# trustbloc/fabric-mod

Measured on AMD Instinct MI355X. Metric: ECDSA P-256 verifies/sec (whole node), higher is better.
Workload: dtype int64; 1 GPU; BASELINE.json configs[1]: block of 10000 tx x 3 endorsements = 30000 P-256 tuples per GPU, verify-only kernel via the C ABI, fresh keypair per signatu; tuples_per_gpu=30000, tx_per_block=10000, endorsements_per_tx=3, seed=20260921, parallelism=1 block per GPU, clock_warmup_launches=100

## Files before the change

### fabric-mod_amd/csrc/fabgpu_api.hip

```cpp
#include <hip/hip_runtime.h>
#include <stdlib.h>
#include <string.h>

#include <algorithm>
#include <atomic>
#include <chrono>
#include <memory>
#include <sys/mman.h>
#include <set>
#include <mutex>
#include <new>
#include <map>
#include <string>
#include <thread>
#include <vector>

#include "../../include/fabgpu.h"
#include "kernels.h"
#include "block_walk_dev.h"
#include "worker_pool.h"
#include "bn_tables29.h"
#include "p256_tables29.h"

using namespace fab;
// ... 77 lines not shown
        cap = want;
        return FABGPU_OK;
    }
    void release() {
        if (h && is_huge) pinned_huge_free(h);
        else if (h) hipHostFree(h);
        h = nullptr;
        cap = 0;
        is_huge = false;
    }
};

}

struct fabgpu_ctx {
    int device = 0;
    bool allow_pair = true;
    bool allow_quad = true;
    bool nym_side_stream = true;
    std::atomic<bool> test_nym_side_after{false};
    bool nym_two_phase = true;
    bool allow_wide = true;
    int pair_table_lds = -1;
    hipStream_t stream = nullptr;
    int fault = 0;
    int32_t* d_gtab = nullptr;
    std::mutex mu;
    Buf fields;
    Buf arena;
    Buf offs;
    Buf out;
    hipEvent_t ev0 = nullptr, ev1 = nullptr;
    bool timed = false;
    bool time_kernels = false;
    struct QWs {
        void* p = nullptr;
        size_t bytes = 0;
        hipEvent_t done = nullptr;
        bool reserved = false;
        bool armed = false;
        NymSide nym_side;
        hipStream_t last = nullptr;
    };
    std::vector<QWs> qws;
    std::mutex kmu;
    std::vector<int32_t*> ktabs;
// ... 155 lines not shown
const char* fabgpu_strerror(int code) {
    switch (code) {
        case FABGPU_OK: return "ok";
        case FABGPU_EINVAL: return "invalid argument";
        case FABGPU_ENODEV: return "no usable gfx950 device (HIP runtime/device unavailable); fall back to bccsp/sw";
        case FABGPU_ENOMEM: return "host or device allocation failed";
        case FABGPU_ELAUNCH: return "HIP launch/copy/execution failure";
        case FABGPU_ETOOBIG: return "batch or arena exceeds 32-bit offsets";
        default: return "unknown fabgpu error";
    }
}

int fabgpu_device_count(fabgpu_ctx*) {
    int n = 0;
    if (hipGetDeviceCount(&n) != hipSuccess) return FABGPU_ENODEV;
    return n;
}

int fabgpu_init(const fabgpu_cfg* cfg, fabgpu_ctx** out) {
    if (!out) return FABGPU_EINVAL;
    *out = nullptr;
    if (cfg && (cfg->flags & ~(uint32_t)(FABGPU_FLAG_ONE_LANE_ONLY | FABGPU_FLAG_TIME_KERNELS | FABGPU_FLAG_NO_QUAD | FABGPU_FLAG_PAIR_TABLE_LDS |
                                          FABGPU_FLAG_PAIR_TABLE_GLOBAL | FABGPU_FLAG_NO_WIDE | FABGPU_FLAG_NYM_FUSED_HASH | FABGPU_FLAG_NYM_NO_SIDE_STREAM |
                                          FABGPU_FLAG_KEY_TABLES_16BIT)) != 0) return FABGPU_EINVAL;
    if (cfg && (cfg->flags & FABGPU_FLAG_PAIR_TABLE_LDS) && (cfg->flags & FABGPU_FLAG_PAIR_TABLE_GLOBAL)) return FABGPU_EINVAL;
    int ndev = 0;
    if (hipGetDeviceCount(&ndev) != hipSuccess || ndev <= 0) return FABGPU_ENODEV;
    int dev = cfg ? cfg->device : -1;
    if (dev < 0) {
        if (hipGetDevice(&dev) != hipSuccess) return FABGPU_ENODEV;
    }
    if (dev >= ndev) return FABGPU_EINVAL;
    hipDeviceProp_t prop;
    if (hipGetDeviceProperties(&prop, dev) != hipSuccess) return FABGPU_ENODEV;
    if (strncmp(prop.gcnArchName, "gfx950", 6) != 0) return FABGPU_ENODEV;
    fabgpu_ctx* ctx = new (std::nothrow) fabgpu_ctx();
    if (!ctx) return FABGPU_ENOMEM;
    ctx->device = dev;
    ctx->walk_map.flags = hipHostMallocMapped | hipHostMallocCoherent;
    ctx->allow_pair = !(cfg && (cfg->flags & FABGPU_FLAG_ONE_LANE_ONLY));
    ctx->allow_quad = !(cfg && (cfg->flags & FABGPU_FLAG_NO_QUAD));
    ctx->nym_two_phase = !(cfg && (cfg->flags & FABGPU_FLAG_NYM_FUSED_HASH));
    ctx->nym_side_stream = !(cfg && (cfg->flags & FABGPU_FLAG_NYM_NO_SIDE_STREAM));
    ctx->key_tables_16 = cfg && (cfg->flags & FABGPU_FLAG_KEY_TABLES_16BIT);
    ctx->allow_wide = ctx->allow_pair && !(cfg && (cfg->flags & FABGPU_FLAG_NO_WIDE));
    ctx->pair_table_lds = cfg && (cfg->flags & FABGPU_FLAG_PAIR_TABLE_LDS) ? 1 : (cfg && (cfg->flags & FABGPU_FLAG_PAIR_TABLE_GLOBAL) ? 0 : pair_table_default());
    if (std::max<size_t>(prop.sharedMemPerBlock, prop.maxSharedMemoryPerMultiProcessor) < pair_table_lds_bytes()) ctx->pair_table_lds = 0;
    ctx->time_kernels = cfg && (cfg->flags & FABGPU_FLAG_TIME_KERNELS);
    DeviceGuard g(dev);
    int rc = FABGPU_OK;
    do {
        if (hipStreamCreateWithFlags(&ctx->stream, hipStreamNonBlocking) != hipSuccess) { rc = FABGPU_ENODEV; break; }
        if (hipStreamCreateWithFlags(&ctx->stream2, hipStreamNonBlocking) != hipSuccess) { rc = FABGPU_ENODEV; break; }
        if (hipEventCreateWithFlags(&ctx->ev_up, hipEventDisableTiming) != hipSuccess) { rc = FABGPU_ENODEV; break; }
        if (hipStreamCreateWithFlags(&ctx->stream3, hipStreamNonBlocking) != hipSuccess) { rc = FABGPU_ENODEV; break; }
        if (hipStreamCreateWithFlags(&ctx->stream4, hipStreamNonBlocking) != hipSuccess) { rc = FABGPU_ENODEV; break; }
        if (hipStreamCreateWithFlags(&ctx->stream_copy, hipStreamNonBlocking) != hipSuccess) { rc = FABGPU_ENODEV; break; }
        {
            bool ok = true;
            for (auto& sc : ctx->stream_copy_more) ok = ok && hipStreamCreateWithFlags(&sc, hipStreamNonBlocking) == hipSuccess;
            if (!ok) { rc = FABGPU_ENODEV; break; }
        }
        {
            bool ok = true;
            for (auto& e : ctx->ev_w) ok = ok && hipEventCreateWithFlags(&e, hipEventDisableTiming) == hipSuccess;
            if (!ok) { rc = FABGPU_ENODEV; break; }
        }
        if (const char* fi = getenv("FABGPU_FAULT_INJECT")) ctx->fault = !strcmp(fi, "launch") ? 1 : (!strcmp(fi, "oom") ? 2 : 0);
        if (hipEventCreate(&ctx->ev0) != hipSuccess || hipEventCreate(&ctx->ev1) != hipSuccess) { rc = FABGPU_ENODEV; break; }
        if (hipMalloc((void**)&ctx->d_gtab, sizeof(int32_t) * GTab16::TABLE_WORDS) != hipSuccess) { rc = FABGPU_ENOMEM; break; }
// ... 111 lines not shown
}
float fab::ctx_last_kernel_ms(fabgpu_ctx* ctx) {
    if (!ctx || !ctx->timed) return -1.0f;
    DeviceGuard g(ctx->device);
    if (hipEventSynchronize(ctx->ev1) != hipSuccess) return -1.0f;
    float ms = -1.0f;
    if (hipEventElapsedTime(&ms, ctx->ev0, ctx->ev1) != hipSuccess) return -1.0f;
    return ms;
}
extern "C" {

int fabgpu_p256_verify_batch_dev(fabgpu_ctx* ctx, size_t n, const void* qx, const void* qy, const void* e, const void* r,
                                 const void* s, void* verdict_bits, void* status, void* stream) {
    if (!ctx || (n && (!qx || !qy || !e || !r || !s || !verdict_bits))) return FABGPU_EINVAL;
    if (n > 0xFFFFFFF0ull) return FABGPU_ETOOBIG;
    if (n == 0) return FABGPU_OK;
    DeviceGuard g(ctx->device);
    hipStream_t st = (hipStream_t)stream;
    size_t wi = 0;
    void* wsp = nullptr;
    int rc = ctx->acquire_qws(verify_workspace_bytes((uint32_t)n, ctx->allow_pair), &wi, &wsp, st);
    if (rc != FABGPU_OK) return rc;
    if (ctx->time_kernels) hipEventRecord(ctx->ev0, st);
    hipError_t err = launch_p256_verify((uint32_t)n, qx, qy, e, r, s, ctx->d_gtab, wsp, verdict_bits, status, ctx->allow_pair, st, 0, ctx->pair_table_lds);
    if (ctx->time_kernels) hipEventRecord(ctx->ev1, st);
    ctx->release_qws(wi, st);
    ctx->timed = ctx->time_kernels;
    return hip_to_rc(launched(ctx, err));
}

int fabgpu_sha256_batch_dev(fabgpu_ctx* ctx, size_t n, const void* arena, size_t arena_bytes, const void* off, void* digests,
                            void* stream) {
    if (!ctx || (n && (!arena || !off || !digests))) return FABGPU_EINVAL;
    if (n > 0xFFFFFFF0ull || arena_bytes > 0xFFFFFFFFull) return FABGPU_ETOOBIG;
    if (n == 0) return FABGPU_OK;
    DeviceGuard g(ctx->device);
    hipStream_t st = (hipStream_t)stream;
    if (ctx->time_kernels) hipEventRecord(ctx->ev0, st);
    hipError_t err = launch_sha256_batch((uint32_t)n, arena, arena_bytes, off, digests, st);
    if (ctx->time_kernels) hipEventRecord(ctx->ev1, st);
    ctx->timed = ctx->time_kernels;
    return hip_to_rc(launched(ctx, err));
}

int fabgpu_sha256_p256_verify_batch_dev(fabgpu_ctx* ctx, size_t n, const void* arena, size_t arena_bytes, const void* off,
                                        const void* qx, const void* qy, const void* r, const void* s, void* verdict_bits,
                                        void* status, void* stream) {
// ... 1842 lines not shown
        if (keyed) {
            e = launch_sha256_p256_verify_keyed(n, sl->d, arena_bytes, a.off2 + 2 * (size_t)row0, a.key_id + row0, nkeys, (const void*)kt, a.r + 32 * (size_t)row0,
                                                a.s + 32 * (size_t)row0, ctx->d_gtab, bits, dt + o_dst + row0, pair, p, ls);
        } else {
            size_t wi = 0;
            void* wsp = nullptr;
            int r2 = ctx->acquire_qws(verify_workspace_bytes(n, pair), &wi, &wsp, ls);
            if (r2 != FABGPU_OK) return r2;
            e = launch_sha256_p256_verify(n, sl->d, arena_bytes, a.off2 + 2 * (size_t)row0, a.qx + 32 * (size_t)row0, a.qy + 32 * (size_t)row0,
                                          a.r + 32 * (size_t)row0, a.s + 32 * (size_t)row0, ctx->d_gtab, wsp, bits, dt + o_dst + row0, pair, p, ls);
            ctx->release_qws(wi, ls);
        }
        return hip_to_rc(e);
    };
    auto verify_creators = [&](bool keyed) -> int {
        hipError_t e;
        if (keyed) {
            e = launch_p256_verify_keyed(tot.creators, a.key_id, nkeys, (const void*)kt, dt + o_dig, a.r, a.s, ctx->d_gtab, dt + o_bitc, dt + o_dst, true, s2, exclusive ? 84u << 10 : 0u);
        } else {
            size_t wi = 0;
            void* wsp = nullptr;
            int r2 = ctx->acquire_qws(verify_workspace_bytes(tot.creators, true), &wi, &wsp, s2);
            if (r2 != FABGPU_OK) return r2;
            e = launch_p256_verify(tot.creators, a.qx, a.qy, dt + o_dig, a.r, a.s, ctx->d_gtab, wsp, dt + o_bitc, dt + o_dst, true, s2, exclusive ? 84u << 10 : 0u, ctx->pair_table_lds);
            ctx->release_qws(wi, s2);
        }
        return hip_to_rc(e);
    };
    auto finish = [&]() -> int {
        if (++ctx->walk_seq == 0) ++ctx->walk_seq;
        ho.seq = ctx->walk_seq;
        if (err == hipSuccess && nym_ran) err = hipStreamWaitEvent(st, ctx->ev_w[6], 0);
        if (err == hipSuccess && memo) err = hipMemsetAsync(dt + o_mslots, 0, (size_t)out.memo_slot_cap * 4, st);
        if (err == hipSuccess && memo) err = hipMemsetAsync(&((WalkMemoTotals*)(dt + o_mtot))->live, 0, 4, st);
        mark("finish: memsets queued");
        if (!memo && !out.tuples && !out.tuple_digest && !out.tuple_qxy && !(has_nym_rows && out.nym_issuer) && walk_small_finish_fits(a, nc)) {
            if (err == hipSuccess) err = launch_walk_status_finish_small(a, nc, ho, st);
            mark("finish: last kernel queued");
            if (err != hipSuccess) return hip_to_rc(err);
            int r2 = wait_host_flag((const uint32_t*)(mh + m_finflag), ho.seq, st);
            if (r2 != FABGPU_OK) return r2;
            rq.summary = *(const WalkSummary*)(mh + m_sum);
            return FABGPU_OK;
        }
        if (err == hipSuccess) err = launch_walk_status_checks(a, nc, st);
        if (memo) {
            if (err == hipSuccess) err = launch_walk_memo_late(a, st);
// ... 335 lines not shown
```

### fabric-mod_amd/csrc/gputest.hip

```cpp
#include <hip/hip_runtime.h>
#include <stdint.h>

#include <vector>

#include "p256_pair29.h"
#include "pair29_bn_gcn.h"
#include "p256_tables29.h"
#include "bn_nym29.h"
#include "bn_quad29.h"
#include "bn_tables29.h"
#include "device_common.h"

using namespace fab;

__global__ void __launch_bounds__(64, 1) gputest_pair_kernel(int op, const int32_t* __restrict__ in, int32_t* __restrict__ out) {
    const int32_t* p = in + threadIdx.x * 36;
    pair_pt P;
    fe C, D;
    for (int i = 0; i < 9; i++) {
        P.A.v[i] = p[i];
        P.B.v[i] = p[9 + i];
        C.v[i] = p[18 + i];
        D.v[i] = p[27 + i];
    }
// ... 277 lines not shown
    hipEventCreate(&e0);
    hipEventCreate(&e1);
    hipLaunchKernelGGL(gputest_mac_ceiling_kernel, dim3(cus), dim3(threads), 0, 0, iters / 16 + 1, 12345u, d);
    hipDeviceSynchronize();
    hipEventRecord(e0, 0);
    hipLaunchKernelGGL(gputest_mac_ceiling_kernel, dim3(cus), dim3(threads), 0, 0, iters, 12345u, d);
    hipEventRecord(e1, 0);
    int rc = hipEventSynchronize(e1) == hipSuccess ? 0 : 4;
    float ms = 0;
    hipEventElapsedTime(&ms, e0, e1);
    std::vector<uint64_t> h(waves);
    if (rc == 0 && hipMemcpy(h.data(), d, sizeof(uint64_t) * waves, hipMemcpyDeviceToHost) != hipSuccess) rc = 5;
    double sum = 0;
    for (uint64_t v : h) sum += (double)v;
    out4[0] = ms;
    out4[1] = sum / waves;
    out4[2] = (double)waves * 64.0 * 64.0 * (double)iters;
    out4[3] = waves;
    hipEventDestroy(e0);
    hipEventDestroy(e1);
    hipFree(d);
    return rc;
}
```

### fabric-mod_amd/csrc/kernels.h

```cpp
#pragma once
#include <hip/hip_runtime_api.h>
#include <stddef.h>
#include <stdint.h>

namespace fab {
constexpr int KTAB_STRIDE = 2;
constexpr int VERIFY_BLOCK = 256;
constexpr int VERIFY_MAX_WGS = 256;
constexpr int VERIFY_PAIR_MAX = 32768;
constexpr size_t QWS_UINT4_PER_LANE = (size_t)16 * 8;
constexpr size_t QWS_PAIR_UINT4_PER_SIG = (size_t)16 * 8;

struct ShaPrefixArgs {
    uint32_t m = 0;
    const void* pre_off = nullptr;
    const void* pre_idx = nullptr;
    void* mid_scratch = nullptr;
    bool spans = false;
    void* digests = nullptr;
    bool mid_ready = false;
    uint32_t lds_reserve = 0;
};
struct VerifyGeom {
    uint32_t block;
    uint32_t wgs;
    bool pair;
};
VerifyGeom verify_geom(uint32_t n, bool allow_pair);
size_t verify_workspace_bytes(uint32_t n, bool allow_pair);
int pair_table_default();
size_t pair_table_lds_bytes();
constexpr int PAIR_TABLE_LDS_FROM = 16384;
hipError_t launch_sha256_midstates(const void* arena, size_t arena_bytes, const ShaPrefixArgs& pa, hipStream_t st);
hipError_t launch_sha256_batch(uint32_t n, const void* arena, size_t arena_bytes, const void* off, void* digests, hipStream_t st, uint32_t lds_spread = 0);
hipError_t launch_sha256_spans(uint32_t n, const void* arena, size_t arena_bytes, const void* spans, void* digests, hipStream_t st,
                               uint32_t lds_reserve = 0, uint32_t lds_spread = 0);
hipError_t launch_gather_sha256(uint32_t n, const void* arena, size_t arena_bytes, const void* spans, const void* out_off, void* scratch,
                                size_t scratch_bytes, void* digests, hipStream_t st, uint32_t lds_reserve = 0, uint32_t lds_spread = 0);
hipError_t launch_p256_verify(uint32_t n, const void* qx, const void* qy, const void* e, const void* r, const void* s,
                              const void* gtab, void* qws, void* verdict_bits, void* status, bool allow_pair, hipStream_t st,
                              uint32_t lds_reserve = 0, int table_lds = 0);
hipError_t launch_sha256_p256_verify(uint32_t n, const void* arena, size_t arena_bytes, const void* off, const void* qx,
                                     const void* qy, const void* r, const void* s, const void* gtab, void* qws,
                                     void* verdict_bits, void* status, bool allow_pair, const ShaPrefixArgs& pa, hipStream_t st);
hipError_t launch_p256_verify_keyed(uint32_t n, const void* key_id, uint32_t nkeys, const void* ktabs, const void* e, const void* r, const void* s,
                                    const void* gtab, void* verdict_bits, void* status, bool allow_pair, hipStream_t st, uint32_t lds_reserve = 0);
hipError_t launch_sha256_p256_verify_keyed(uint32_t n, const void* arena, size_t arena_bytes, const void* off, const void* key_id, uint32_t nkeys,
                                           const void* ktabs, const void* r, const void* s, const void* gtab, void* verdict_bits, void* status,
                                           bool allow_pair, const ShaPrefixArgs& pa, hipStream_t st);

constexpr int WIDE_LAUNCH_MAX = 8192;
constexpr size_t WIDE_SCRATCH_BYTES = 144;
constexpr uint32_t SPREAD_NONE = 0xFFFFFFFFu;
uint32_t spread_waves_per_cu(uint32_t wavefronts);
hipError_t launch_p256_wide_pre(uint32_t n, const void* key_id, uint32_t nkeys, const void* ktabs, const void* r, const void* s, const void* gtab,
                                void* scratch, hipStream_t st, uint32_t lds_spread = 0);
hipError_t launch_p256_wide_post(uint32_t n, const void* e, const void* r, const void* gtab, const void* scratch, void* verdict_bits, void* status,
                                 hipStream_t st, uint32_t lds_spread = 0);
hipError_t launch_sha256_messages(uint32_t n, const void* arena, size_t arena_bytes, const void* off, const ShaPrefixArgs& pa, hipStream_t st);
constexpr uint32_t SHA_COOP_MAX = 2048;
hipError_t launch_sha256_mixed(uint32_t n, const void* arena, size_t arena_bytes, const void* off, bool pairs, void* digests, hipStream_t st,
                               uint32_t lds_reserve = 0);
hipError_t launch_sha256_messages_coop(uint32_t n, const void* arena, size_t arena_bytes, const void* off, const ShaPrefixArgs& pa, hipStream_t st,
                                       uint32_t lds_spread = 0);
// ... 32 lines not shown
```

### fabric-mod_amd/csrc/kernels.hip

```cpp
#include <hip/hip_runtime.h>
#include <stdlib.h>
#include <stdint.h>

#include "device_common.h"
#include "kernels.h"
#include "p256_pair29.h"

namespace fab {


__global__ void __launch_bounds__(256) sha256_midstate_kernel(uint32_t m, const uint32_t* __restrict__ arena32, uint32_t arena_words,
                                                               const uint32_t* __restrict__ pre_off, uint32_t spans, uint32_t* __restrict__ mid) {
    uint32_t p = blockIdx.x * blockDim.x + threadIdx.x;
    bool active = p < m;
    uint32_t pc = active ? p : (m - 1);
    uint32_t start = pre_off[spans ? 2 * pc : pc], len = pre_off[spans ? 2 * pc + 1 : pc + 1] - start;
    uint32_t nfull = active ? (len >> 6) : 0, maxfull = nfull;
#pragma unroll
    for (int o = 32; o >= 1; o >>= 1) {
        uint32_t other = __shfl_xor(maxfull, o, 64);
        maxfull = other > maxfull ? other : maxfull;
    }
    maxfull = __builtin_amdgcn_readfirstlane(maxfull);
    uint32_t h[8];
// ... 59 lines not shown
                                                                         uint8_t* __restrict__ status) {
    constexpr int NP = BLOCK / 2;
    const bool odd = (threadIdx.x & 1) != 0;
    const uint32_t pairidx = threadIdx.x >> 1;
    PairQTab<NP> qtab = PairQTab<NP>::of(qws + (size_t)blockIdx.x * (QWS_PAIR_UINT4_PER_SIG * NP), pairidx);
    uint32_t* verdict32 = reinterpret_cast<uint32_t*>(verdict_bits);
    const uint32_t ntiles = (n + NP - 1) / NP;
    for (uint32_t tile = blockIdx.x; tile < ntiles; tile += gridDim.x) {
        uint32_t i = tile * NP + pairidx;
        bool active = i < n;
        uint32_t ic = active ? i : (n - 1);
        u256 vqx, vqy, ve, vr, vs;
        load_be_field(vqx, qx, ic);
        load_be_field(vqy, qy, ic);
        load_be_field(ve, e, ic);
        load_be_field(vr, r, ic);
        load_be_field(vs, s, ic);
        uint32_t st = p256_verify_pair29(vqx, vqy, ve, vr, vs, gtab, qtab, odd);
        pair_emit_verdict(i, n, active, odd, st, verdict32, status);
    }
}

template <int BLOCK>
__global__ void __launch_bounds__(BLOCK, 1) p256_verify_pair_lds_kernel(uint32_t n, const uint8_t* __restrict__ qx, const uint8_t* __restrict__ qy,
                                                                             const uint8_t* __restrict__ e, const uint8_t* __restrict__ r,
                                                                             const uint8_t* __restrict__ s, const int32_t* __restrict__ gtab,
                                                                             uint64_t* __restrict__ verdict_bits, uint8_t* __restrict__ status) {
    extern __shared__ uint4 pair_lds[];
    constexpr int NP = BLOCK / 2;
    const bool odd = (threadIdx.x & 1) != 0;
    const uint32_t pairidx = threadIdx.x >> 1;
    PairQTabLds qtab = PairQTabLds::of(pair_lds, pairidx);
    uint32_t* verdict32 = reinterpret_cast<uint32_t*>(verdict_bits);
    const uint32_t ntiles = (n + NP - 1) / NP;
    for (uint32_t tile = blockIdx.x; tile < ntiles; tile += gridDim.x) {
        uint32_t i = tile * NP + pairidx;
        bool active = i < n;
        uint32_t ic = active ? i : (n - 1);
        u256 vqx, vqy, ve, vr, vs;
        load_be_field(vqx, qx, ic);
        load_be_field(vqy, qy, ic);
        load_be_field(ve, e, ic);
        load_be_field(vr, r, ic);
        load_be_field(vs, s, ic);
        uint32_t st = p256_verify_pair29<PairQTabLds, 4>(vqx, vqy, ve, vr, vs, gtab, qtab, odd);
        pair_emit_verdict(i, n, active, odd, st, verdict32, status);
    }
}

template <int BLOCK>
__global__ void __launch_bounds__(BLOCK, 2) p256_verify_keyed_kernel(uint32_t n, const uint32_t* __restrict__ key_id, uint32_t nkeys,
                                                                          const int32_t* const* __restrict__ ktabs, const uint8_t* __restrict__ e,
                                                                          const uint8_t* __restrict__ r, const uint8_t* __restrict__ s,
                                                                          const int32_t* __restrict__ gtab, uint64_t* __restrict__ verdict_bits,
                                                                          uint8_t* __restrict__ status) {
    GTab16 gt{gtab};
    const uint32_t ntiles = (n + BLOCK - 1) / BLOCK;
    for (uint32_t tile = blockIdx.x; tile < ntiles; tile += gridDim.x) {
        uint32_t i = tile * BLOCK + threadIdx.x;
        bool active = i < n;
        uint32_t ic = active ? i : (n - 1);
        uint32_t kid = key_id[ic];
        bool kok = kid < nkeys;
        KeyTab8 kt{ktabs[KTAB_STRIDE * (size_t)(kok ? kid : 0)]};
        const int32_t* kt16 = ktabs[KTAB_STRIDE * (size_t)(kok ? kid : 0) + 1];
        u256 ve, vr, vs;
        load_be_field(ve, e, ic);
        load_be_field(vr, r, ic);
        load_be_field(vs, s, ic);
// ... 217 lines not shown
}
hipError_t launch_gather_sha256(uint32_t n, const void* arena, size_t arena_bytes, const void* spans, const void* out_off, void* scratch,
                                size_t scratch_bytes, void* digests, hipStream_t st, uint32_t lds_reserve, uint32_t lds_spread) {
    if (n == 0) return hipSuccess;
    dim3 grid((n + 3) / 4), block(256);
    hipLaunchKernelGGL(gather_spans_kernel, grid, block, lds_reserve, st, n, (const uint8_t*)arena, (uint32_t)arena_bytes, (const uint32_t*)spans,
                       (const uint32_t*)out_off, (uint8_t*)scratch);
    hipError_t e = hipGetLastError();
    if (e != hipSuccess) return e;
    if (lds_reserve) return launch_sha256_mixed(n, scratch, scratch_bytes, out_off, false, digests, st, lds_reserve);
    return launch_sha256_batch(n, scratch, scratch_bytes, out_off, digests, st, lds_spread);
}

VerifyGeom verify_geom(uint32_t n, bool allow_pair) {
    VerifyGeom g;
    g.block = VERIFY_BLOCK;
    g.pair = allow_pair && n <= (uint32_t)VERIFY_PAIR_MAX;
    uint32_t per_wg = g.pair ? VERIFY_BLOCK / 2 : VERIFY_BLOCK;
    uint32_t tiles = (n + per_wg - 1) / per_wg;
    g.wgs = tiles < (uint32_t)VERIFY_MAX_WGS ? tiles : (uint32_t)VERIFY_MAX_WGS;
    return g;
}
int pair_table_default() { return -1; }
size_t pair_table_lds_bytes() { return (size_t)(VERIFY_BLOCK / 2) * PAIR_LDS_CELLS_PER_SIG * 16; }
size_t verify_workspace_bytes(uint32_t n, bool allow_pair) {
    VerifyGeom g = verify_geom(n, allow_pair);
    if (g.pair) return (size_t)g.wgs * (g.block / 2) * QWS_PAIR_UINT4_PER_SIG * 16;
    return (size_t)g.wgs * g.block * QWS_UINT4_PER_LANE * 16;
}
hipError_t launch_p256_verify(uint32_t n, const void* qx, const void* qy, const void* e, const void* r, const void* s,
                              const void* gtab, void* qws, void* verdict_bits, void* status, bool allow_pair, hipStream_t st, uint32_t lds_reserve, int table_lds) {
    if (n == 0) return hipSuccess;
    VerifyGeom g = verify_geom(n, allow_pair);
    dim3 grid(g.wgs), block(g.block);
    if (table_lds < 0) table_lds = n > (uint32_t)PAIR_TABLE_LDS_FROM ? 1 : 0;
    if (g.pair && table_lds) {
        hipLaunchKernelGGL(p256_verify_pair_lds_kernel<VERIFY_BLOCK>, grid, block, (size_t)(VERIFY_BLOCK / 2) * PAIR_LDS_CELLS_PER_SIG * 16, st, n, (const uint8_t*)qx,
                           (const uint8_t*)qy, (const uint8_t*)e, (const uint8_t*)r, (const uint8_t*)s, (const int32_t*)gtab, (uint64_t*)verdict_bits, (uint8_t*)status);
        return hipGetLastError();
    }
    if (g.pair) {
        hipLaunchKernelGGL(p256_verify_pair_kernel<VERIFY_BLOCK>, grid, block, lds_reserve, st, n, (const uint8_t*)qx, (const uint8_t*)qy, (const uint8_t*)e,
                           (const uint8_t*)r, (const uint8_t*)s, (const int32_t*)gtab, (uint4*)qws, (uint64_t*)verdict_bits, (uint8_t*)status);
        return hipGetLastError();
    }
    hipLaunchKernelGGL(p256_verify_kernel<VERIFY_BLOCK>, grid, block, lds_reserve, st, n, (const uint8_t*)qx, (const uint8_t*)qy, (const uint8_t*)e,
                       (const uint8_t*)r, (const uint8_t*)s, (const int32_t*)gtab, (uint4*)qws, (uint64_t*)verdict_bits, (uint8_t*)status);
    return hipGetLastError();
}
hipError_t launch_sha256_p256_verify(uint32_t n, const void* arena, size_t arena_bytes, const void* off, const void* qx,
                                     const void* qy, const void* r, const void* s, const void* gtab, void* qws,
                                     void* verdict_bits, void* status, bool allow_pair, const ShaPrefixArgs& pa, hipStream_t st) {
    if (n == 0) return hipSuccess;
    sha_prefixes pre = launch_midstates(arena, arena_bytes, pa, st);
    VerifyGeom g = verify_geom(n, allow_pair);
    dim3 grid(g.wgs), block(g.block);
    if (g.pair) {
        hipLaunchKernelGGL(sha256_p256_verify_pair_kernel<VERIFY_BLOCK>, grid, block, pa.lds_reserve, st, n, (const uint32_t*)arena, (uint32_t)((arena_bytes + 3) / 4),
                           (const uint32_t*)off, (const uint8_t*)qx, (const uint8_t*)qy, (const uint8_t*)r, (const uint8_t*)s,
                           (const int32_t*)gtab, (uint4*)qws, (uint64_t*)verdict_bits, (uint8_t*)status, pre);
// ... 21 lines not shown

hipError_t launch_sha256_p256_verify_keyed(uint32_t n, const void* arena, size_t arena_bytes, const void* off, const void* key_id, uint32_t nkeys,
                                           const void* ktabs, const void* r, const void* s, const void* gtab, void* verdict_bits, void* status,
                                           bool allow_pair, const ShaPrefixArgs& pa, hipStream_t st) {
    if (n == 0) return hipSuccess;
    sha_prefixes pre = launch_midstates(arena, arena_bytes, pa, st);
    VerifyGeom g = verify_geom(n, allow_pair);
    dim3 grid(g.wgs), block(g.block);
    if (g.pair)
        hipLaunchKernelGGL(sha256_p256_verify_keyed_pair_kernel<VERIFY_BLOCK>, grid, block, pa.lds_reserve, st, n, (const uint32_t*)arena,
                           (uint32_t)((arena_bytes + 3) / 4), (const uint32_t*)off, (const uint32_t*)key_id, nkeys, (const int32_t* const*)ktabs,
                           (const uint8_t*)r, (const uint8_t*)s, (const int32_t*)gtab, (uint64_t*)verdict_bits, (uint8_t*)status, pre);
    else
        hipLaunchKernelGGL(sha256_p256_verify_keyed_kernel<VERIFY_BLOCK>, grid, block, pa.lds_reserve, st, n, (const uint32_t*)arena,
                           (uint32_t)((arena_bytes + 3) / 4), (const uint32_t*)off, (const uint32_t*)key_id, nkeys, (const int32_t* const*)ktabs,
                           (const uint8_t*)r, (const uint8_t*)s, (const int32_t*)gtab, (uint64_t*)verdict_bits, (uint8_t*)status, pre);
    return hipGetLastError();
}

int warm_kernel_functions_kernels() {
    int ok = 0;
    hipFuncAttributes a;
    const void* fns[] = {(const void*)p256_verify_kernel<VERIFY_BLOCK>, (const void*)p256_verify_pair_kernel<VERIFY_BLOCK>,
                         (const void*)p256_verify_pair_lds_kernel<VERIFY_BLOCK>, (const void*)p256_verify_keyed_kernel<VERIFY_BLOCK>,
                         (const void*)p256_verify_keyed_pair_kernel<VERIFY_BLOCK>, (const void*)sha256_p256_verify_keyed_kernel<VERIFY_BLOCK>,
                         (const void*)sha256_p256_verify_keyed_pair_kernel<VERIFY_BLOCK>, (const void*)sha256_p256_verify_pair_kernel<VERIFY_BLOCK>,
                         (const void*)sha256_p256_verify_kernel<VERIFY_BLOCK>, (const void*)sha256_midstate_kernel, (const void*)gather_spans_kernel};
    for (const void* f : fns) ok += hipFuncGetAttributes(&a, f) == hipSuccess ? 1 : 0;
    return ok;
}

}
```

### fabric-mod_amd/csrc/p256_pair29.h

```cpp
#pragma once
#include "p256_verify29.h"
#include "pair29_gcn.h"

namespace fab {

struct pair_pt {
    fe A, B;
};

__device__ __forceinline__ int32_t pair_swap_i32(int32_t v) {
    return __builtin_amdgcn_update_dpp(0, v, 0xB1, 0xF, 0xF, false);
}
__device__ __forceinline__ void pair_swap_fe(fe& r, const fe& a) {
#pragma unroll
    for (int i = 0; i < 9; i++) r.v[i] = pair_swap_i32(a.v[i]);
}
__device__ __forceinline__ void pair_sel(pair_pt& r, bool c, const pair_pt& a, const pair_pt& b) {
    fe_sel(r.A, c, a.A, b.A);
    fe_sel(r.B, c, a.B, b.B);
}

#define PAIR_TMPS __attribute__((unused)) fe tU1, tU2, tU3, tU4, tU6, tW, tH, tRR, tP1, tP2, tT0, tT1, tTD
#define PAIR_DBL(P) PAIR29_DBL((P).A, (P).B, tU1, tU2, tU3, tW, tP1, tP2, tT0, tT1, tTD)
#define PAIR_ADD(R, P, C, D) PAIR29_ADD((R).A, (R).B, (P).A, (P).B, tH, tRR, tW, tU1, tU2, tU3, tU4, tU6, tP1, tP2, tT0, tT1, tTD, C, D)
// ... 245 lines not shown
    pair_pt Rp;
    PAIR_ADD(Rp, S, C, D);
    bool hz = fe_is_zero(tH);
    bool rz_own = fe_is_zero(tRR);
    int32_t rz_other = pair_swap_i32(rz_own ? 1 : 0);
    bool rz = odd ? (rz_other != 0) : rz_own;
    r_inf = t_inf & s_inf;
    bool use_T = s_inf & !t_inf;
    bool use_S = t_inf & !s_inf;
    bool both = !s_inf & !t_inf;
    bool use_dbl = both & hz & rz;
    r_inf = r_inf | (both & hz & !rz);
    Rr = Rp;
    if (__any(use_dbl)) {
        pair_pt Rd = T;
        PAIR_DBL(Rd);
        pair_sel(Rr, use_dbl, Rd, Rr);
    }
    pair_sel(Rr, use_T, T, Rr);
    pair_sel(Rr, use_S, S, Rr);
}

template <class QTab, int W = 5>
__device__ __forceinline__ void pair_combined_mult29(pair_pt& Rr, bool& r_inf, const u256& u1, const u256& u2, const fe& QX, const fe& QY,
                                                     const int32_t* __restrict__ gtab, const QTab& qtab, bool odd) {
    static_assert(W == 4 || W == 5, "signed 4- or 5-bit windows");
    constexpr int TAB = 1 << (W - 1);
    constexpr int NWIN = (257 + W - 1) / W;
    const fe ONE = {FE29_R1};
    PAIR_TMPS;
    pair_pt Qp;
    Qp.A = QX;
    fe_sel(Qp.B, odd, ONE, QY);

    qtab.store_state(1, Qp, odd);
#pragma unroll 1
    for (int j = 2; j <= TAB; j += 2) {
        pair_pt d;
        qtab.load_state((uint32_t)(j >> 1), d, odd);
        PAIR_DBL(d);
        qtab.store_state(j, d, odd);
        if (j < TAB) {
            pair_pt d1;
            PAIR_MADD(d1, d, QX, QY);
            qtab.store_state(j + 1, d1, odd);
        }
    }

    uint32_t kw[9];
#pragma unroll
    for (int i = 0; i < 8; i++) kw[i] = u2.w[i];
    kw[8] = 0;
    pair_pt T = Qp;
    bool t_inf = true;
#pragma unroll 1
    for (int i = NWIN - 1; i >= 0; i--) {
        uint32_t field;
        if (i == 0) {
            field = (kw[0] << 1) & ((2u << W) - 1u);
        } else {
            int p = W * i - 1;
            uint64_t two = ((uint64_t)kw[(p >> 5) + 1] << 32) | kw[p >> 5];
            field = (uint32_t)(two >> (p & 31)) & ((2u << W) - 1u);
        }
        int32_t digit = (int32_t)((field >> 1) & (uint32_t)(TAB - 1)) + (int32_t)(field & 1u) - (int32_t)((field >> W) << (W - 1));
        bool neg = digit < 0;
        uint32_t mag = (uint32_t)(neg ? -digit : digit);
        fe C, D;
        qtab.load_crossed(mag ? mag : 1u, C, D, odd);
        if (i != NWIN - 1) {
#pragma unroll 1
            for (int k = 0; k < W; k++) PAIR_DBL(T);
        }
        {
            const int32_t nm = neg ? -1 : 0, nc = neg ? 1 : 0;
#pragma unroll
            for (int l = 0; l < 9; l++) D.v[l] = (D.v[l] ^ nm) + nc;
// ... 9 lines not shown
            pair_swap_fe(sc, C);
            pair_swap_fe(sd, D);
            ent.A = sc;
            fe_sel(ent.B, odd, sc, sd);
            pair_sel(T, take_ent, ent, T);
        }
        t_inf = t_inf & (mag == 0);
    }
    if (W == 4) {
        const u256 NM2 = {{0xFC63254Fu, 0xF3B9CAC2u, 0xA7179E84u, 0xBCE6FAADu, 0xFFFFFFFFu, 0xFFFFFFFFu, 0x00000000u, 0xFFFFFFFFu}};
        bool special = true;
#pragma unroll
        for (int l = 0; l < 8; l++) special = special & (u2.w[l] == NM2.w[l]);
        if (__any(special)) {
            pair_pt two;
            qtab.load_state(2u, two, odd);
            fe ny;
#pragma unroll
            for (int l = 0; l < 9; l++) ny.v[l] = -two.B.v[l];
            fe_sel(two.B, odd, two.B, ny);
            pair_sel(T, special, two, T);
        }
    }

    pair_pt S;
    bool s_inf;
    pair_comb_mult29<GTab16>(S, s_inf, u1, gtab, Qp, odd);
    pair_final_add29(Rr, r_inf, S, s_inf, T, t_inf, odd);
}

template <class KTab = KeyTab8>
__device__ __forceinline__ void pair_combined_mult_keyed29(pair_pt& Rr, bool& r_inf, const u256& u1, const u256& u2,
                                                           const int32_t* __restrict__ gtab, const int32_t* __restrict__ ktab, bool odd) {
    const fe ONE = {FE29_R1};
    fe gx, gy;
    GTab16 gt{gtab};
    gt.load(0, 1u, gx, gy);
    pair_pt seed, S, T;
    seed.A = gx;
    fe_sel(seed.B, odd, ONE, gy);
    bool s_inf, t_inf;
    pair_comb_mult29<KTab>(T, t_inf, u2, ktab, seed, odd);
    pair_comb_mult29<GTab16>(S, s_inf, u1, gtab, seed, odd);
    pair_final_add29(Rr, r_inf, S, s_inf, T, t_inf, odd);
}

// ... 35 lines not shown

    pair_pt Rr;
    bool r_inf;
    pair_combined_mult29<QTab, W>(Rr, r_inf, u1, u2, QX, QY, gtab, qtab, odd);
    bool ok = pair_x_equals_r29(Rr, r_inf, r);
    uint32_t st = ok ? ST_VALID : ST_BAD_MATH;
    return early != ST_VALID ? early : st;
}

__device__ __forceinline__ uint32_t p256_verify_keyed_pair29(const u256& e, const u256& r, const u256& s, const int32_t* __restrict__ gtab,
                                                              const int32_t* __restrict__ ktab, const int32_t* __restrict__ ktab16, bool odd) {
    uint32_t early = range_status(r, s);
    u256 u1, u2;
    pair_ecdsa_scalars29(u1, u2, e, r, s, odd);
    pair_pt Rr;
    bool r_inf;
    if (__all(ktab16 != nullptr)) pair_combined_mult_keyed29<GTab16>(Rr, r_inf, u1, u2, gtab, ktab16, odd);
    else pair_combined_mult_keyed29<KeyTab8>(Rr, r_inf, u1, u2, gtab, ktab, odd);
    bool ok = pair_x_equals_r29(Rr, r_inf, r);
    uint32_t st = ok ? ST_VALID : ST_BAD_MATH;
    return early != ST_VALID ? early : st;
}

}
```

### fabric-mod_amd/fabgpu/__init__.py

```python
from __future__ import annotations

import ctypes
import os
from typing import List, Optional, Sequence, Tuple

import numpy as np

_HERE = os.path.dirname(os.path.abspath(__file__))
_LIB_PATH = os.environ.get("FABGPU_LIB_PATH") or os.path.join(os.path.dirname(_HERE), "lib", "libfabgpu.so")

FABGPU_OK = 0
FABGPU_EINVAL = -1
FLAG_ONE_LANE_ONLY = 1
FLAG_TIME_KERNELS = 2
FLAG_NYM_NO_SIDE_STREAM = 128
FLAG_NYM_FUSED_HASH = 64
FLAG_NO_QUAD = 4
FLAG_PAIR_TABLE_LDS = 8
FLAG_PAIR_TABLE_GLOBAL = 16
FLAG_KEY_TABLES_16BIT = 256
FLAG_NO_WIDE = 32
ST_VALID, ST_BAD_MATH, ST_HIGH_S, ST_RANGE, ST_OFF_CURVE = 0, 1, 2, 3, 4

_u8p = ctypes.POINTER(ctypes.c_uint8)
_u32p = ctypes.POINTER(ctypes.c_uint32)
_u64p = ctypes.POINTER(ctypes.c_uint64)
_vp = ctypes.c_void_p
_sz = ctypes.c_size_t


class FabgpuError(RuntimeError):
    """Infrastructure failure (non-zero FABGPU_E*): the Go provider would fall back to bccsp/sw."""


class BCCSPError(Exception):
    """A non-nil Go `error` from the provider (same text as bccsp/sw)."""


class _IdBatch(ctypes.Structure):
    _fields_ = [("n", ctypes.c_size_t), ("arena", ctypes.c_void_p), ("arena_bytes", ctypes.c_size_t), ("off", ctypes.c_void_p),
                ("n_prefixes", ctypes.c_uint32), ("pre_off", ctypes.c_void_p), ("pre_idx", ctypes.c_void_p), ("qx", ctypes.c_void_p),
                ("qy", ctypes.c_void_p), ("key_id", ctypes.c_void_p), ("r", ctypes.c_void_p), ("s", ctypes.c_void_p),
# ... 1051 lines not shown
```

### include/fabgpu.h

```cpp
#ifndef FABGPU_H
#define FABGPU_H

#include <stddef.h>
#include <stdint.h>

#ifdef __cplusplus
extern "C" {
#endif

#define FABGPU_ABI_VERSION 6

#define FABGPU_OK 0
#define FABGPU_EINVAL (-1)
#define FABGPU_ENODEV (-2)
#define FABGPU_ENOMEM (-3)
#define FABGPU_ELAUNCH (-4)
#define FABGPU_ETOOBIG (-5)

#define FABGPU_ST_VALID 0
#define FABGPU_ST_BAD_MATH 1
#define FABGPU_ST_HIGH_S 2
#define FABGPU_ST_RANGE 3
#define FABGPU_ST_OFF_CURVE 4

typedef struct fabgpu_ctx fabgpu_ctx;

#define FABGPU_FLAG_ONE_LANE_ONLY 1u
#define FABGPU_FLAG_NO_QUAD 4u
#define FABGPU_FLAG_TIME_KERNELS 2u
#define FABGPU_FLAG_PAIR_TABLE_LDS 8u
#define FABGPU_FLAG_PAIR_TABLE_GLOBAL 16u
#define FABGPU_FLAG_NO_WIDE 32u

#define FABGPU_FLAG_NYM_FUSED_HASH 64u
#define FABGPU_FLAG_NYM_NO_SIDE_STREAM 128u

#define FABGPU_FLAG_KEY_TABLES_16BIT 256u

typedef struct fabgpu_cfg {
    int32_t device;
    uint32_t max_batch;
    uint32_t max_arena;
    uint32_t flags;
} fabgpu_cfg;

int fabgpu_init(const fabgpu_cfg* cfg, fabgpu_ctx** out);
void fabgpu_shutdown(fabgpu_ctx* ctx);
int fabgpu_device_count(fabgpu_ctx* ctx);
const char* fabgpu_strerror(int code);
int fabgpu_abi_version(void);

int fabgpu_p256_verify_batch(fabgpu_ctx* ctx, size_t n, const uint8_t* qx, const uint8_t* qy, const uint8_t* e,
                             const uint8_t* r, const uint8_t* s, uint64_t* verdict_bits, uint8_t* status);

int fabgpu_sha256_batch(fabgpu_ctx* ctx, size_t n, const uint8_t* arena, const uint32_t* off, uint8_t* digests);

int fabgpu_sha256_p256_verify_batch(fabgpu_ctx* ctx, size_t n, const uint8_t* arena, const uint32_t* off,
                                    const uint8_t* qx, const uint8_t* qy, const uint8_t* r, const uint8_t* s,
// ... 104 lines not shown
```

Before: 51.53 million verifies/s.

## Split pair LDS verify kernel into helper and main wave groups

The default LDS-table pair verify kernel now launches twice as many threads per workgroup. Helper waves compute the ECDSA scalars and the fixed-base comb multiplication u1·G, while main waves decode Q, build the Q window table and run the u2·Q ladder. The two groups hand off u2 and the partial point S through an added LDS region, separated by two block barriers. The aim is to run the G and Q multiplications concurrently instead of one after the other per lane. In exchange it costs more LDS and threads per workgroup, the wave groups carry uneven work, and it risks lower occupancy. The old single-group kernel stays available behind a new PAIR_SOLO flag, and a wave-placement test kernel is added.

```diff
diff --git a/fabric-mod_amd/csrc/fabgpu_api.hip b/fabric-mod_amd/csrc/fabgpu_api.hip
--- a/fabric-mod_amd/csrc/fabgpu_api.hip
+++ b/fabric-mod_amd/csrc/fabgpu_api.hip
@@ -123,6 +123,7 @@
     bool nym_two_phase = true;
     bool allow_wide = true;
     int pair_table_lds = -1;
+    bool pair_solo = false;
     hipStream_t stream = nullptr;
     int fault = 0;
     int32_t* d_gtab = nullptr;
@@ -324,7 +325,7 @@
     *out = nullptr;
     if (cfg && (cfg->flags & ~(uint32_t)(FABGPU_FLAG_ONE_LANE_ONLY | FABGPU_FLAG_TIME_KERNELS | FABGPU_FLAG_NO_QUAD | FABGPU_FLAG_PAIR_TABLE_LDS |
                                           FABGPU_FLAG_PAIR_TABLE_GLOBAL | FABGPU_FLAG_NO_WIDE | FABGPU_FLAG_NYM_FUSED_HASH | FABGPU_FLAG_NYM_NO_SIDE_STREAM |
-                                          FABGPU_FLAG_KEY_TABLES_16BIT)) != 0) return FABGPU_EINVAL;
+                                          FABGPU_FLAG_KEY_TABLES_16BIT | FABGPU_FLAG_PAIR_SOLO)) != 0) return FABGPU_EINVAL;
     if (cfg && (cfg->flags & FABGPU_FLAG_PAIR_TABLE_LDS) && (cfg->flags & FABGPU_FLAG_PAIR_TABLE_GLOBAL)) return FABGPU_EINVAL;
     int ndev = 0;
     if (hipGetDeviceCount(&ndev) != hipSuccess || ndev <= 0) return FABGPU_ENODEV;
@@ -347,7 +348,9 @@
     ctx->key_tables_16 = cfg && (cfg->flags & FABGPU_FLAG_KEY_TABLES_16BIT);
     ctx->allow_wide = ctx->allow_pair && !(cfg && (cfg->flags & FABGPU_FLAG_NO_WIDE));
     ctx->pair_table_lds = cfg && (cfg->flags & FABGPU_FLAG_PAIR_TABLE_LDS) ? 1 : (cfg && (cfg->flags & FABGPU_FLAG_PAIR_TABLE_GLOBAL) ? 0 : pair_table_default());
-    if (std::max<size_t>(prop.sharedMemPerBlock, prop.maxSharedMemoryPerMultiProcessor) < pair_table_lds_bytes()) ctx->pair_table_lds = 0;
+    ctx->pair_solo = cfg && (cfg->flags & FABGPU_FLAG_PAIR_SOLO);
+    if (std::max<size_t>(prop.sharedMemPerBlock, prop.maxSharedMemoryPerMultiProcessor) < (ctx->pair_solo ? pair_table_lds_solo_bytes() : pair_table_lds_bytes()))
+        ctx->pair_table_lds = 0;
     ctx->time_kernels = cfg && (cfg->flags & FABGPU_FLAG_TIME_KERNELS);
     DeviceGuard g(dev);
     int rc = FABGPU_OK;
@@ -505,7 +508,7 @@
     int rc = ctx->acquire_qws(verify_workspace_bytes((uint32_t)n, ctx->allow_pair), &wi, &wsp, st);
     if (rc != FABGPU_OK) return rc;
     if (ctx->time_kernels) hipEventRecord(ctx->ev0, st);
-    hipError_t err = launch_p256_verify((uint32_t)n, qx, qy, e, r, s, ctx->d_gtab, wsp, verdict_bits, status, ctx->allow_pair, st, 0, ctx->pair_table_lds);
+    hipError_t err = launch_p256_verify((uint32_t)n, qx, qy, e, r, s, ctx->d_gtab, wsp, verdict_bits, status, ctx->allow_pair, st, 0, ctx->pair_table_lds, ctx->pair_solo);
     if (ctx->time_kernels) hipEventRecord(ctx->ev1, st);
     ctx->release_qws(wi, st);
     ctx->timed = ctx->time_kernels;
@@ -2394,7 +2397,8 @@
             void* wsp = nullptr;
             int r2 = ctx->acquire_qws(verify_workspace_bytes(tot.creators, true), &wi, &wsp, s2);
             if (r2 != FABGPU_OK) return r2;
-            e = launch_p256_verify(tot.creators, a.qx, a.qy, dt + o_dig, a.r, a.s, ctx->d_gtab, wsp, dt + o_bitc, dt + o_dst, true, s2, exclusive ? 84u << 10 : 0u, ctx->pair_table_lds);
+            e = launch_p256_verify(tot.creators, a.qx, a.qy, dt + o_dig, a.r, a.s, ctx->d_gtab, wsp, dt + o_bitc, dt + o_dst, true, s2, exclusive ? 84u << 10 : 0u, ctx->pair_table_lds,
+                                   ctx->pair_solo);
             ctx->release_qws(wi, s2);
         }
         return hip_to_rc(e);
diff --git a/fabric-mod_amd/csrc/gputest.hip b/fabric-mod_amd/csrc/gputest.hip
--- a/fabric-mod_amd/csrc/gputest.hip
+++ b/fabric-mod_amd/csrc/gputest.hip
@@ -323,3 +323,22 @@
     hipFree(d);
     return rc;
 }
+
+__global__ void __launch_bounds__(512, 1) gputest_wave_placement_kernel(uint32_t* __restrict__ out) {
+    extern __shared__ uint32_t placement_lds[];
+    const uint32_t id = __builtin_amdgcn_s_getreg((31 << 11) | 4);
+    placement_lds[threadIdx.x] = id;
+    __syncthreads();
+    if ((threadIdx.x & 63) == 0) out[blockIdx.x * 8 + (threadIdx.x >> 6)] = placement_lds[threadIdx.x];
+}
+
+extern "C" int gputest_wave_placement(uint32_t wgs, uint32_t lds_bytes, uint32_t* out) {
+    if (!out || wgs == 0 || lds_bytes < 512 * 4) return 1;
+    uint32_t* d = nullptr;
+    if (hipMalloc(&d, sizeof(uint32_t) * 8 * wgs) != hipSuccess) return 3;
+    hipLaunchKernelGGL(gputest_wave_placement_kernel, dim3(wgs), dim3(512), lds_bytes, 0, d);
+    int rc = hipGetLastError() == hipSuccess && hipDeviceSynchronize() == hipSuccess ? 0 : 4;
+    if (rc == 0 && hipMemcpy(out, d, sizeof(uint32_t) * 8 * wgs, hipMemcpyDeviceToHost) != hipSuccess) rc = 5;
+    hipFree(d);
+    return rc;
+}
diff --git a/fabric-mod_amd/csrc/kernels.h b/fabric-mod_amd/csrc/kernels.h
--- a/fabric-mod_amd/csrc/kernels.h
+++ b/fabric-mod_amd/csrc/kernels.h
@@ -30,6 +30,7 @@
 size_t verify_workspace_bytes(uint32_t n, bool allow_pair);
 int pair_table_default();
 size_t pair_table_lds_bytes();
+size_t pair_table_lds_solo_bytes();
 constexpr int PAIR_TABLE_LDS_FROM = 16384;
 hipError_t launch_sha256_midstates(const void* arena, size_t arena_bytes, const ShaPrefixArgs& pa, hipStream_t st);
 hipError_t launch_sha256_batch(uint32_t n, const void* arena, size_t arena_bytes, const void* off, void* digests, hipStream_t st, uint32_t lds_spread = 0);
@@ -39,7 +40,8 @@
                                 size_t scratch_bytes, void* digests, hipStream_t st, uint32_t lds_reserve = 0, uint32_t lds_spread = 0);
 hipError_t launch_p256_verify(uint32_t n, const void* qx, const void* qy, const void* e, const void* r, const void* s,
                               const void* gtab, void* qws, void* verdict_bits, void* status, bool allow_pair, hipStream_t st,
-                              uint32_t lds_reserve = 0, int table_lds = 0);
+                              uint32_t lds_reserve = 0, int table_lds = 0,
+                              bool pair_solo = false);
 hipError_t launch_sha256_p256_verify(uint32_t n, const void* arena, size_t arena_bytes, const void* off, const void* qx,
                                      const void* qy, const void* r, const void* s, const void* gtab, void* qws,
                                      void* verdict_bits, void* status, bool allow_pair, const ShaPrefixArgs& pa, hipStream_t st);
diff --git a/fabric-mod_amd/csrc/kernels.hip b/fabric-mod_amd/csrc/kernels.hip
--- a/fabric-mod_amd/csrc/kernels.hip
+++ b/fabric-mod_amd/csrc/kernels.hip
@@ -105,7 +105,7 @@
 }
 
 template <int BLOCK>
-__global__ void __launch_bounds__(BLOCK, 1) p256_verify_pair_lds_kernel(uint32_t n, const uint8_t* __restrict__ qx, const uint8_t* __restrict__ qy,
+__global__ void __launch_bounds__(BLOCK, 1) p256_verify_pair_lds_solo_kernel(uint32_t n, const uint8_t* __restrict__ qx, const uint8_t* __restrict__ qy,
                                                                              const uint8_t* __restrict__ e, const uint8_t* __restrict__ r,
                                                                              const uint8_t* __restrict__ s, const int32_t* __restrict__ gtab,
                                                                              uint64_t* __restrict__ verdict_bits, uint8_t* __restrict__ status) {
@@ -128,6 +128,59 @@
         load_be_field(vs, s, ic);
         uint32_t st = p256_verify_pair29<PairQTabLds, 4>(vqx, vqy, ve, vr, vs, gtab, qtab, odd);
         pair_emit_verdict(i, n, active, odd, st, verdict32, status);
+    }
+}
+
+template <int BLOCK>
+__global__ void __launch_bounds__(2 * BLOCK, 1) p256_verify_pair_lds_kernel(uint32_t n, const uint8_t* __restrict__ qx, const uint8_t* __restrict__ qy,
+                                                                                 const uint8_t* __restrict__ e, const uint8_t* __restrict__ r,
+                                                                                 const uint8_t* __restrict__ s, const int32_t* __restrict__ gtab,
+                                                                                 uint64_t* __restrict__ verdict_bits, uint8_t* __restrict__ status) {
+    extern __shared__ uint4 pair_lds[];
+    constexpr int NP = BLOCK / 2;
+    const bool helper = __builtin_amdgcn_readfirstlane(threadIdx.x) >= (uint32_t)BLOCK;
+    const uint32_t lane = threadIdx.x & (uint32_t)(BLOCK - 1);
+    const bool odd = (lane & 1) != 0;
+    const uint32_t pairidx = lane >> 1;
+    PairQTabLds qtab = PairQTabLds::of(pair_lds, pairidx);
+    const PairHandoffLds<BLOCK> hand = PairHandoffLds<BLOCK>::of(reinterpret_cast<uint32_t*>(pair_lds + NP * PAIR_LDS_CELLS_PER_SIG), lane);
+    uint32_t* verdict32 = reinterpret_cast<uint32_t*>(verdict_bits);
+    const uint32_t ntiles = (n + NP - 1) / NP;
+    for (uint32_t tile = blockIdx.x; tile < ntiles; tile += gridDim.x) {
+        uint32_t i = tile * NP + pairidx;
+        bool active = i < n;
+        uint32_t ic = active ? i : (n - 1);
+        u256 u1;
+        uint32_t early = 0;
+        pair_pt Qp, T;
+        bool q_ok = false, t_inf = true;
+        if (helper) {
+            u256 ve, vr, vs;
+            load_be_field(ve, e, ic);
+            load_be_field(vr, r, ic);
+            load_be_field(vs, s, ic);
+            pair_helper_scalars29(u1, early, ve, vr, vs, hand, odd);
+        } else {
+            u256 vqx, vqy;
+            load_be_field(vqx, qx, ic);
+            load_be_field(vqy, qy, ic);
+            q_ok = pair_main_table29(Qp, vqx, vqy, qtab, odd);
+        }
+        __syncthreads();
+        if (helper) {
+            pair_helper_comb29(u1, early, gtab, hand, odd);
+        } else {
+            u256 u2;
+            hand.get_u2(u2);
+            pair_u2_mult29<PairQTabLds, 4>(T, t_inf, u2, Qp, qtab, odd);
+        }
+        __syncthreads();
+        if (!helper) {
+            u256 vr;
+            load_be_field(vr, r, ic);
+            uint32_t st = pair_main_finish29(T, t_inf, q_ok, vr, hand, odd);
+            pair_emit_verdict(i, n, active, odd, st, verdict32, status);
+        }
     }
 }
 
@@ -391,20 +444,27 @@
     return g;
 }
 int pair_table_default() { return -1; }
-size_t pair_table_lds_bytes() { return (size_t)(VERIFY_BLOCK / 2) * PAIR_LDS_CELLS_PER_SIG * 16; }
+size_t pair_table_lds_bytes() { return (size_t)(VERIFY_BLOCK / 2) * PAIR_LDS_CELLS_PER_SIG * 16 + (size_t)VERIFY_BLOCK * PAIR_HAND_WORDS * 4; }
+size_t pair_table_lds_solo_bytes() { return (size_t)(VERIFY_BLOCK / 2) * PAIR_LDS_CELLS_PER_SIG * 16; }
 size_t verify_workspace_bytes(uint32_t n, bool allow_pair) {
     VerifyGeom g = verify_geom(n, allow_pair);
     if (g.pair) return (size_t)g.wgs * (g.block / 2) * QWS_PAIR_UINT4_PER_SIG * 16;
     return (size_t)g.wgs * g.block * QWS_UINT4_PER_LANE * 16;
 }
 hipError_t launch_p256_verify(uint32_t n, const void* qx, const void* qy, const void* e, const void* r, const void* s,
-                              const void* gtab, void* qws, void* verdict_bits, void* status, bool allow_pair, hipStream_t st, uint32_t lds_reserve, int table_lds) {
+                              const void* gtab, void* qws, void* verdict_bits, void* status, bool allow_pair, hipStream_t st, uint32_t lds_reserve, int table_lds,
+                              bool pair_solo) {
     if (n == 0) return hipSuccess;
     VerifyGeom g = verify_geom(n, allow_pair);
     dim3 grid(g.wgs), block(g.block);
     if (table_lds < 0) table_lds = n > (uint32_t)PAIR_TABLE_LDS_FROM ? 1 : 0;
+    if (g.pair && table_lds && !pair_solo) {
+        hipLaunchKernelGGL(p256_verify_pair_lds_kernel<VERIFY_BLOCK>, grid, dim3(2 * VERIFY_BLOCK), pair_table_lds_bytes(), st, n, (const uint8_t*)qx,
+                           (const uint8_t*)qy, (const uint8_t*)e, (const uint8_t*)r, (const uint8_t*)s, (const int32_t*)gtab, (uint64_t*)verdict_bits, (uint8_t*)status);
+        return hipGetLastError();
+    }
     if (g.pair && table_lds) {
-        hipLaunchKernelGGL(p256_verify_pair_lds_kernel<VERIFY_BLOCK>, grid, block, (size_t)(VERIFY_BLOCK / 2) * PAIR_LDS_CELLS_PER_SIG * 16, st, n, (const uint8_t*)qx,
+        hipLaunchKernelGGL(p256_verify_pair_lds_solo_kernel<VERIFY_BLOCK>, grid, block, pair_table_lds_solo_bytes(), st, n, (const uint8_t*)qx,
                            (const uint8_t*)qy, (const uint8_t*)e, (const uint8_t*)r, (const uint8_t*)s, (const int32_t*)gtab, (uint64_t*)verdict_bits, (uint8_t*)status);
         return hipGetLastError();
     }
@@ -472,7 +532,8 @@
     int ok = 0;
     hipFuncAttributes a;
     const void* fns[] = {(const void*)p256_verify_kernel<VERIFY_BLOCK>, (const void*)p256_verify_pair_kernel<VERIFY_BLOCK>,
-                         (const void*)p256_verify_pair_lds_kernel<VERIFY_BLOCK>, (const void*)p256_verify_keyed_kernel<VERIFY_BLOCK>,
+                         (const void*)p256_verify_pair_lds_kernel<VERIFY_BLOCK>, (const void*)p256_verify_pair_lds_solo_kernel<VERIFY_BLOCK>,
+                         (const void*)p256_verify_keyed_kernel<VERIFY_BLOCK>,
                          (const void*)p256_verify_keyed_pair_kernel<VERIFY_BLOCK>, (const void*)sha256_p256_verify_keyed_kernel<VERIFY_BLOCK>,
                          (const void*)sha256_p256_verify_keyed_pair_kernel<VERIFY_BLOCK>, (const void*)sha256_p256_verify_pair_kernel<VERIFY_BLOCK>,
                          (const void*)sha256_p256_verify_kernel<VERIFY_BLOCK>, (const void*)sha256_midstate_kernel, (const void*)gather_spans_kernel};
diff --git a/fabric-mod_amd/csrc/p256_pair29.h b/fabric-mod_amd/csrc/p256_pair29.h
--- a/fabric-mod_amd/csrc/p256_pair29.h
+++ b/fabric-mod_amd/csrc/p256_pair29.h
@@ -291,17 +291,9 @@
 }
 
 template <class QTab, int W = 5>
-__device__ __forceinline__ void pair_combined_mult29(pair_pt& Rr, bool& r_inf, const u256& u1, const u256& u2, const fe& QX, const fe& QY,
-                                                     const int32_t* __restrict__ gtab, const QTab& qtab, bool odd) {
-    static_assert(W == 4 || W == 5, "signed 4- or 5-bit windows");
+__device__ __forceinline__ void pair_qtab_build29(const pair_pt& Qp, const fe& QX, const fe& QY, const QTab& qtab, bool odd) {
     constexpr int TAB = 1 << (W - 1);
-    constexpr int NWIN = (257 + W - 1) / W;
-    const fe ONE = {FE29_R1};
     PAIR_TMPS;
-    pair_pt Qp;
-    Qp.A = QX;
-    fe_sel(Qp.B, odd, ONE, QY);
-
     qtab.store_state(1, Qp, odd);
 #pragma unroll 1
     for (int j = 2; j <= TAB; j += 2) {
@@ -315,13 +307,19 @@
             qtab.store_state(j + 1, d1, odd);
         }
     }
-
+}
+
+template <class QTab, int W = 5>
+__device__ __forceinline__ void pair_u2_mult29(pair_pt& T, bool& t_inf, const u256& u2, const pair_pt& Qp, const QTab& qtab, bool odd) {
+    constexpr int TAB = 1 << (W - 1);
+    constexpr int NWIN = (257 + W - 1) / W;
+    PAIR_TMPS;
     uint32_t kw[9];
 #pragma unroll
     for (int i = 0; i < 8; i++) kw[i] = u2.w[i];
     kw[8] = 0;
-    pair_pt T = Qp;
-    bool t_inf = true;
+    T = Qp;
+    t_inf = true;
 #pragma unroll 1
     for (int i = NWIN - 1; i >= 0; i--) {
         uint32_t field;
@@ -377,6 +375,20 @@
             pair_sel(T, special, two, T);
         }
     }
+}
+
+template <class QTab, int W = 5>
+__device__ __forceinline__ void pair_combined_mult29(pair_pt& Rr, bool& r_inf, const u256& u1, const u256& u2, const fe& QX, const fe& QY,
+                                                     const int32_t* __restrict__ gtab, const QTab& qtab, bool odd) {
+    static_assert(W == 4 || W == 5, "signed 4- or 5-bit windows");
+    const fe ONE = {FE29_R1};
+    pair_pt Qp;
+    Qp.A = QX;
+    fe_sel(Qp.B, odd, ONE, QY);
+    pair_qtab_build29<QTab, W>(Qp, QX, QY, qtab, odd);
+    pair_pt T;
+    bool t_inf;
+    pair_u2_mult29<QTab, W>(T, t_inf, u2, Qp, qtab, odd);
 
     pair_pt S;
     bool s_inf;
@@ -458,4 +470,92 @@
     return early != ST_VALID ? early : st;
 }
 
-}
+constexpr int PAIR_HAND_U2_WORDS = 8;
+constexpr int PAIR_HAND_S_WORDS = 9 + 9 + 1;
+constexpr int PAIR_HAND_WORDS = PAIR_HAND_U2_WORDS + PAIR_HAND_S_WORDS;
+
+template <int LANES>
+struct PairHandoffLds {
+    uint32_t* u2;
+    uint32_t* s;
+    static __device__ __forceinline__ PairHandoffLds of(uint32_t* base, uint32_t lane) {
+        return PairHandoffLds{base + lane, base + PAIR_HAND_U2_WORDS * LANES + lane};
+    }
+    __device__ __forceinline__ void put_u2(const u256& v) const {
+#pragma unroll
+        for (int w = 0; w < 8; w++) u2[w * LANES] = v.w[w];
+    }
+    __device__ __forceinline__ void get_u2(u256& v) const {
+#pragma unroll
+        for (int w = 0; w < 8; w++) v.w[w] = u2[w * LANES];
+    }
+    __device__ __forceinline__ void put_s(const pair_pt& S, bool s_inf, uint32_t early) const {
+#pragma unroll
+        for (int l = 0; l < 9; l++) s[l * LANES] = (uint32_t)S.A.v[l];
+#pragma unroll
+        for (int l = 0; l < 9; l++) s[(9 + l) * LANES] = (uint32_t)S.B.v[l];
+        s[18 * LANES] = (s_inf ? 1u : 0u) | (early << 1);
+    }
+    __device__ __forceinline__ void get_s(pair_pt& S, bool& s_inf, uint32_t& early) const {
+#pragma unroll
+        for (int l = 0; l < 9; l++) S.A.v[l] = (int32_t)s[l * LANES];
+#pragma unroll
+        for (int l = 0; l < 9; l++) S.B.v[l] = (int32_t)s[(9 + l) * LANES];
+        uint32_t f = s[18 * LANES];
+        s_inf = (f & 1u) != 0;
+        early = f >> 1;
+    }
+};
+
+template <class Hand>
+__device__ __forceinline__ void pair_helper_scalars29(u256& u1, uint32_t& early, const u256& e, const u256& r, const u256& s, const Hand& hand,
+                                                      bool odd) {
+    early = range_status(r, s);
+    u256 u2;
+    pair_ecdsa_scalars29(u1, u2, e, r, s, odd);
+    hand.put_u2(u2);
+}
+
+template <class Hand>
+__device__ __forceinline__ void pair_helper_comb29(const u256& u1, uint32_t early, const int32_t* __restrict__ gtab, const Hand& hand, bool odd) {
+    const fe ONE = {FE29_R1};
+    fe gx, gy;
+    GTab16 gt{gtab};
+    gt.load(0, 1u, gx, gy);
+    pair_pt seed, S;
+    seed.A = gx;
+    fe_sel(seed.B, odd, ONE, gy);
+    bool s_inf;
+    pair_comb_mult29<GTab16>(S, s_inf, u1, gtab, seed, odd);
+    hand.put_s(S, s_inf, early);
+}
+
+template <class QTab>
+__device__ __forceinline__ bool pair_main_table29(pair_pt& Qp, const u256& qx, const u256& qy, const QTab& qtab, bool odd) {
+    const u256 P = FAB_P256_P;
+    const fe ONE = {FE29_R1};
+    bool q_in_field = lt256(qx, P) & lt256(qy, P);
+    fe QX, QY;
+    fe_to_mont(QX, qx);
+    fe_to_mont(QY, qy);
+    bool q_ok = q_in_field & on_curve29(QX, QY);
+    Qp.A = QX;
+    fe_sel(Qp.B, odd, ONE, QY);
+    pair_qtab_build29<QTab, 4>(Qp, QX, QY, qtab, odd);
+    return q_ok;
+}
+
+template <class Hand>
+__device__ __forceinline__ uint32_t pair_main_finish29(const pair_pt& T, bool t_inf, bool q_ok, const u256& r, const Hand& hand, bool odd) {
+    pair_pt S, Rr;
+    bool s_inf, r_inf;
+    uint32_t early;
+    hand.get_s(S, s_inf, early);
+    if (early == ST_VALID && !q_ok) early = ST_OFF_CURVE;
+    pair_final_add29(Rr, r_inf, S, s_inf, T, t_inf, odd);
+    bool ok = pair_x_equals_r29(Rr, r_inf, r);
+    uint32_t st = ok ? ST_VALID : ST_BAD_MATH;
+    return early != ST_VALID ? early : st;
+}
+
+}
diff --git a/fabric-mod_amd/fabgpu/__init__.py b/fabric-mod_amd/fabgpu/__init__.py
--- a/fabric-mod_amd/fabgpu/__init__.py
+++ b/fabric-mod_amd/fabgpu/__init__.py
@@ -18,6 +18,7 @@
 FLAG_NO_QUAD = 4
 FLAG_PAIR_TABLE_LDS = 8
 FLAG_PAIR_TABLE_GLOBAL = 16
+FLAG_PAIR_SOLO = 1024
 FLAG_KEY_TABLES_16BIT = 256
 FLAG_NO_WIDE = 32
 ST_VALID, ST_BAD_MATH, ST_HIGH_S, ST_RANGE, ST_OFF_CURVE = 0, 1, 2, 3, 4
diff --git a/include/fabgpu.h b/include/fabgpu.h
--- a/include/fabgpu.h
+++ b/include/fabgpu.h
@@ -34,6 +34,8 @@
 
 #define FABGPU_FLAG_NYM_FUSED_HASH 64u
 #define FABGPU_FLAG_NYM_NO_SIDE_STREAM 128u
+
+#define FABGPU_FLAG_PAIR_SOLO 1024u
 
 #define FABGPU_FLAG_KEY_TABLES_16BIT 256u
 
```

Result: faster. 54.79 million verifies/s (median of 6 runs) (+6.3%).
